# viniciusvidal2/slam-sensor-fusion

Measured on AMD Instinct MI355X. Metric: scans_per_s_200k_scan_vs_10M_map, higher is better.
Workload: dtype f32 points / f64 accumulation

## Files before the change

slam_sensor_fusion_amd/csrc/sf_icp.hip:

```cpp
#include "sf_common.hpp"
#include "sf_nn.hpp"
#include "sf_tile.hpp"
#include "sf_order.hpp"
#include "sf_p2p.hpp"
#include "sf_schedule.hpp"

#include <cfloat>
#include <cstdlib>
#include <cmath>
#include <vector>
#include <mutex>
#include <string>

namespace {

constexpr int BLK = 256;
constexpr int NREC_P2P = 17;
constexpr int NREC_PLANE = 30;
constexpr int REC_STRIDE = 32;

struct IcpState {
    double T[16];
    double rec[REC_STRIDE];
    double fitness, rmse, prev_fitness, prev_rmse;
// ... 454 lines not shown
            }
        }
    }
    return need;
}

struct QueryIn {
    double sx, sy, sz;
    float qx, qy, qz;
    float4 c1, c2;
    float e;
    size_t o;
    bool valid;
};

template <int MODE, bool SHARD>
__device__ __forceinline__ QueryIn query_in(const float *__restrict__ X0x, const float *__restrict__ X0y, const float *__restrict__ X0z, int n, int b, const IcpState *S, float xlo,
                                            float xhi, const uint32_t *__restrict__ own_off, const float4 *__restrict__ qcache, int64_t cache_n, bool cache_live, int slot,
                                            int n_live)
{
    QueryIn q;
    q.sx = q.sy = q.sz = 0.0;
    q.qx = q.qy = q.qz = 0.0f;
    q.c1 = q.c2 = make_float4(0.f, 0.f, 0.f, 0.f);
    q.e = 0.0f;
    q.o = 0;
    q.valid = false;
    if (slot < n_live) {
        const size_t o = SHARD ? (size_t)own_off[b] + (size_t)slot : (size_t)b * n + (size_t)slot;
        q.o = o;
        if (cache_live) {
            q.c1 = qcache[o];
            if (MODE == 2) { q.c2 = qcache[(size_t)cache_n + o]; q.e = q.c2.w; }
            else q.e = reinterpret_cast<const float *>(qcache + (size_t)cache_n)[o];
        }
        const double x0 = X0x[o], y0 = X0y[o], z0 = X0z[o];
        q.sx = S->T[0] * x0 + S->T[1] * y0 + S->T[2] * z0 + S->T[3];
        q.sy = S->T[4] * x0 + S->T[5] * y0 + S->T[6] * z0 + S->T[7];
        q.sz = S->T[8] * x0 + S->T[9] * y0 + S->T[10] * z0 + S->T[11];
        q.qx = (float)q.sx; q.qy = (float)q.sy; q.qz = (float)q.sz;
        q.valid = !SHARD || (q.qx >= xlo && q.qx < xhi);
    }
    return q;
}

__device__ __forceinline__ LanePair make_pair(const QueryIn &q, const sf::NNHit &hit, const float4 &tn)
{
    LanePair P;
    P.sx = q.sx; P.sy = q.sy; P.sz = q.sz;
    P.px = hit.px; P.py = hit.py; P.pz = hit.pz;
    P.tn = tn;
    P.ok = hit.j >= 0;
    return P;
}

template <int MODE>
__device__ __forceinline__ int table_serve(const SfGrid &g, const QueryIn &q, float thr, float m_now, const sf::NNHit &seed, float4 *__restrict__ qcache, int64_t cache_n,
                                            sf::NNHit &hit, float4 &tn)
{
    sf::NNHit th;
    const int stage = sf::nn_research_table(g, q.qx, q.qy, q.qz, thr, seed, th);
    if (stage == 0) return 0;
    const bool same = th.j == seed.j;
    hit = th;
    if (MODE == 2) tn = same ? make_float4(q.c2.x, q.c2.y, q.c2.z, 0.0f) : (th.j >= 0 ? g.nrm[th.j] : make_float4(0.f, 0.f, 0.f, 0.f));
    const float en = fmaxf(sqrtf(th.lb2) * 0.9999f + m_now * 0.999998f - 1.0e-6f, 1.0e-30f);
    if (!same) qcache[q.o] = make_float4(th.px, th.py, th.pz, __int_as_float(th.j));
    if (MODE == 2) qcache[(size_t)cache_n + q.o] = make_float4(tn.x, tn.y, tn.z, en);
    else reinterpret_cast<float *>(qcache + (size_t)cache_n)[q.o] = en;
    return stage;
}

__device__ __forceinline__ void table_count(uint32_t *__restrict__ stats, bool tried, int stage)
{
    const unsigned long long tm = __ballot(tried), sm = __ballot(stage != 0), gm = __ballot(stage == sf::NBR_BY_GAP);
    if ((threadIdx.x & 63) == 0 && tm) {
        uint32_t *sh = stats + NN_STATS_PER * ((blockIdx.x + blockIdx.y * gridDim.x) & (NN_STATS_SHARDS - 1));
        atomicAdd(&sh[2], (uint32_t)__popcll(sm));
        atomicAdd(&sh[3], (uint32_t)__popcll(tm & ~sm));
        atomicAdd(&sh[4], (uint32_t)__popcll(gm));
    }
}

template <int MODE, bool WINDOW, bool SHARD>
__device__ __forceinline__ LanePair nn_pair(const SfGrid &g, const SfWindow &w, const float *__restrict__ X0x, const float *__restrict__ X0y, const float *__restrict__ X0z,
                                            int n, int b, const IcpState *S, float thr, float xlo, float xhi, const uint32_t *__restrict__ own_off,
                                            float4 *__restrict__ qcache, int64_t cache_n, int slot, int n_live, sf::WaveNN *ws, uint32_t *__restrict__ stats,
                                            sf::PhaseClock *pc = nullptr, bool try_table = true)
{
    const bool cache_live = qcache != nullptr && S->cache_live != 0;
    const QueryIn q = query_in<MODE, SHARD>(X0x, X0y, X0z, n, b, S, xlo, xhi, own_off, qcache, cache_n, cache_live, slot, n_live);
    const float qx = q.qx, qy = q.qy, qz = q.qz;
    const size_t o = q.o;
    float *ecache = reinterpret_cast<float *>(qcache + (size_t)cache_n);
    const float m_now = (float)S->motion;
    sf::NNHit hit;
    float4 tn;
    sf::NNHit seed;
    bool need = reuse_certificate(q.valid, qx, qy, qz, thr, m_now, q.e, q.c1, q.c2, hit, tn, seed);
    if constexpr (!WINDOW && !SHARD) {
        if (try_table && g.nbr != nullptr && S->n_research >= g.nbr_from) {
            const bool tried = need && seed.j >= 0;
            int served = 0;
            if (tried) {
                served = table_serve<MODE>(g, q, thr, m_now, seed, qcache, cache_n, hit, tn);
                need = served == 0;
            }
            if (stats) table_count(stats, tried, served);
        }
    }
    const unsigned long long need_mask = __ballot(need);
    if (stats && (threadIdx.x & 63) == 0 && need_mask) {
        uint32_t *sh = stats + NN_STATS_PER * ((blockIdx.x + blockIdx.y * gridDim.x) & (NN_STATS_SHARDS - 1));
        atomicAdd(&sh[0], (uint32_t)__popcll(need_mask));
        atomicAdd(&sh[1], 1u);
    }
    SF_PH(pc, 0);
    if (need_mask != 0ull) {
        const sf::NNHit h = sf::nn_search_wave<WINDOW>(g, w, need, qx, qy, qz, thr, ws, seed, pc);
        if (need) {
            hit = h;
            if (MODE == 2 && h.j >= 0) tn = g.nrm[h.j];
            if (qcache) {
                const float en = fmaxf(sqrtf(h.lb2) * 0.9999f + m_now * 0.999998f - 1.0e-6f, 1.0e-30f);
                qcache[o] = make_float4(h.px, h.py, h.pz, __int_as_float(h.j));
                if (MODE == 2) qcache[(size_t)cache_n + o] = make_float4(tn.x, tn.y, tn.z, en);
                else ecache[o] = en;
            }
        }
    }
    if (qcache && !cache_live && !need && slot < n_live) {
        if (MODE == 2) qcache[(size_t)cache_n + o] = make_float4(0.f, 0.f, 0.f, 0.f);
        else ecache[o] = 0.0f;
    }
    SF_PH(pc, 6);
    return make_pair(q, hit, tn);
}

struct PairTerms { double wgt, ux, uy, uz, tx, ty, tz, ex, ey, ez, d2, r; double J[6]; };
template <int MODE>
__device__ __forceinline__ PairTerms pair_terms(const LanePair &P)
{
    PairTerms t;
    const bool ok = P.ok;
    t.wgt = ok ? 1.0 : 0.0;
    t.ux = ok ? P.sx : 0.0; t.uy = ok ? P.sy : 0.0; t.uz = ok ? P.sz : 0.0;
    t.tx = (double)(ok ? P.px : 0.0f); t.ty = (double)(ok ? P.py : 0.0f); t.tz = (double)(ok ? P.pz : 0.0f);
    t.ex = t.ux - t.tx; t.ey = t.uy - t.ty; t.ez = t.uz - t.tz;
    t.d2 = t.ex * t.ex + t.ey * t.ey + t.ez * t.ez;
    if (MODE == 2) {
        const double nx = (double)(ok ? P.tn.x : 0.0f), ny = (double)(ok ? P.tn.y : 0.0f), nz = (double)(ok ? P.tn.z : 0.0f);
        t.r = t.ex * nx + t.ey * ny + t.ez * nz;
        t.J[0] = t.uy * nz - t.uz * ny; t.J[1] = t.uz * nx - t.ux * nz; t.J[2] = t.ux * ny - t.uy * nx;
        t.J[3] = nx; t.J[4] = ny; t.J[5] = nz;
    } else {
        t.r = 0.0;
#pragma unroll
        for (int a = 0; a < 6; ++a) t.J[a] = 0.0;
    }
    return t;
}

struct RobustArg { int kind; double k; };
__device__ __forceinline__ double robust_weight(const RobustArg &rk, double r)
{
    const double a = fabs(r), k = rk.k;
    switch (rk.kind) {
    case SF_ROBUST_HUBER: return a <= k ? 1.0 : k / a;
    case SF_ROBUST_CAUCHY: { const double q = r / k; return 1.0 / (1.0 + q * q); }
    case SF_ROBUST_TUKEY: { const double q = r / k, s = 1.0 - q * q; return a <= k ? s * s : 0.0; }
    case SF_ROBUST_GM: { const double k2 = k * k, s = k2 / (k2 + r * r); return s * s; }
    default: return 1.0;
    }
}

template <int MODE>
__device__ __forceinline__ void add_half(const PairTerms &t, int h, double (&v)[16])
{
    if (MODE == 1) {
        if (h == 0) {
            v[0] += t.wgt;
            v[1] += t.ux; v[2] += t.uy; v[3] += t.uz;
            v[4] += t.tx; v[5] += t.ty; v[6] += t.tz;
            v[7] = fma(t.ux, t.tx, v[7]); v[8] = fma(t.ux, t.ty, v[8]); v[9] = fma(t.ux, t.tz, v[9]);
            v[10] = fma(t.uy, t.tx, v[10]); v[11] = fma(t.uy, t.ty, v[11]); v[12] = fma(t.uy, t.tz, v[12]);
            v[13] = fma(t.uz, t.tx, v[13]); v[14] = fma(t.uz, t.ty, v[14]); v[15] = fma(t.uz, t.tz, v[15]);
        } else {
            v[0] += t.d2;
        }
    } else {
        if (h == 0) { v[0] += t.wgt; v[1] = fma(t.r, t.r, v[1]); }
        int k = 2;
#pragma unroll
        for (int a = 0; a < 6; ++a) {
#pragma unroll
            for (int c = a; c < 6; ++c) {
                if (h == 0 && k < 16) v[k] = fma(t.J[a], t.J[c], v[k]);
                if (h == 1 && k >= 16) v[k - 16] = fma(t.J[a], t.J[c], v[k - 16]);
                ++k;
            }
        }
        if (h == 1) {
// ... 723 lines not shown
__device__ __forceinline__ constexpr int k6(int a, int b) { return a <= b ? (a == 0 ? b : (a == 1 ? 2 + b : 5)) : (b == 0 ? a : (b == 1 ? 2 + a : 5)); }

struct MomIn { double x[3], n[3], p[3], c, w; };
__device__ __forceinline__ MomIn mom_in(const LanePair &P, bool take)
{
    MomIn t;
    const bool ok = P.ok && take;
    t.w = ok ? 1.0 : 0.0;
    t.x[0] = ok ? P.sx : 0.0; t.x[1] = ok ? P.sy : 0.0; t.x[2] = ok ? P.sz : 0.0;
    t.p[0] = (double)(ok ? P.px : 0.0f); t.p[1] = (double)(ok ? P.py : 0.0f); t.p[2] = (double)(ok ? P.pz : 0.0f);
    t.n[0] = (double)(ok ? P.tn.x : 0.0f); t.n[1] = (double)(ok ? P.tn.y : 0.0f); t.n[2] = (double)(ok ? P.tn.z : 0.0f);
    t.c = t.n[0] * t.p[0] + t.n[1] * t.p[1] + t.n[2] * t.p[2];
    return t;
}
template <int I>
__device__ __forceinline__ double mom_fma(const MomIn &t, double acc)
{
    if constexpr (I < 36) return fma(t.n[k6a(I / 6)] * t.n[k6b(I / 6)], t.x[k6a(I % 6)] * t.x[k6b(I % 6)], acc);
    else if constexpr (I < 54) return fma(t.n[k6a((I - 36) / 3)] * t.n[k6b((I - 36) / 3)], t.x[(I - 36) % 3], acc);
    else if constexpr (I < 60) return fma(t.n[k6a(I - 54)], t.n[k6b(I - 54)], acc);
    else if constexpr (I < 69) return fma(t.c * t.n[(I - 60) / 3], t.x[(I - 60) % 3], acc);
    else if constexpr (I < 72) return fma(t.c, t.n[I - 69], acc);
    else if constexpr (I == 72) return fma(t.c, t.c, acc);
    else if constexpr (I == 73) return acc + t.w;
    else if constexpr (I < 80) return fma(t.x[k6a(I - 74)], t.x[k6b(I - 74)], acc);
    else if constexpr (I < 83) return acc + t.x[I - 80];
    else if constexpr (I < 92) return fma(t.p[(I - 83) / 3], t.x[(I - 83) % 3], acc);
    else if constexpr (I < 95) return acc + t.p[I - 92];
    else return fma(t.p[0], t.p[0], fma(t.p[1], t.p[1], fma(t.p[2], t.p[2], acc)));
}
template <int H, int K = 0>
__device__ __forceinline__ void mom_add16(const MomIn &t, double (&v)[16])
{
    if constexpr (K < 16) {
        v[K] = mom_fma<16 * H + K>(t, v[K]);
        mom_add16<H, K + 1>(t, v);
    }
}

template <bool SHARD>
__device__ __forceinline__ bool stays_frozen(const QueryIn &q, bool in_range, float thr, float m_now, float guard, float xlo, float xhi)
{
    if (!in_range) return true;
    if (!(isfinite(q.qx) && isfinite(q.qy) && isfinite(q.qz))) return true;
    if (SHARD) {
        const float gx = guard * 1.000002f + (fabsf(q.qx) + 1.0f) * 2.6e-7f + 1.0e-6f;
        if (q.valid) {
            if (!(q.qx - gx >= xlo && q.qx + gx < xhi)) return false;
        } else {
            return q.qx + gx < xlo || q.qx - gx >= xhi;
        }
    }
    if (!(q.e > 0.0f)) return false;
    const float m = m_now + guard * 1.000002f;
    const float reach = q.e - m * 1.000002f - (fabsf(q.qx) + fabsf(q.qy) + fabsf(q.qz) + 3.0f * guard + 1.0f) * 2.6e-7f - (q.e + m) * 5.0e-7f - 1.0e-6f;
    const float rt = sqrtf(thr);
    const int32_t jc = __float_as_int(q.c1.w);
    if (jc < 0) return rt * 1.0001f + 1.0e-6f < reach;
    const float d = sqrtf(sf::l2_simple(q.qx, q.qy, q.qz, q.c1.x, q.c1.y, q.c1.z));
    if (!((d + guard) * 1.0001f + 1.0e-6f < reach)) return false;
    const bool stays_in = (d + guard) * 1.0001f + 1.0e-6f < rt * 0.9999f;
    const bool stays_out = (d - guard) * 0.9999f - 1.0e-6f > rt * 1.0001f;
    return stays_in || stays_out;
}

struct FzArgs {
    const float *X0x, *X0y, *X0z;
    int n;
    const IcpState *st;
    float thr, xlo, xhi;
    double *partials;
    int nblocks;
    const uint32_t *own_off;
    float4 *qcache;
    int64_t cache_n;
    uint32_t *stats;
    const FreezeState *fz;
    double *mom_part;
    uint32_t *act_cnt;
    uint16_t *act_ids;
    const uint32_t *act_all;
};

template <int Q, bool SHARD>
__device__ __forceinline__ void nn_red_fz_row(const SfGrid &g, const SfWindow &w, const FzArgs &A, int b, int bx, int fmode)
{
    constexpr int MODE = 2;
    constexpr int NREC = NREC_PLANE;
    static_assert(FZ_CAP == 64 * Q, "wave 0 takes FZ_CAP active queries in Q rounds of 64");
    const float *__restrict__ X0x = A.X0x, *__restrict__ X0y = A.X0y, *__restrict__ X0z = A.X0z;
    const int n = A.n, nblocks = A.nblocks;
    const float thr = A.thr, xlo = A.xlo, xhi = A.xhi;
    double *__restrict__ partials = A.partials, *__restrict__ mom_part = A.mom_part;
    const uint32_t *__restrict__ own_off = A.own_off, *__restrict__ act_all = A.act_all;
    float4 *__restrict__ qcache = A.qcache;
    const int64_t cache_n = A.cache_n;
    uint32_t *__restrict__ stats = A.stats, *__restrict__ act_cnt = A.act_cnt;
    uint16_t *__restrict__ act_ids = A.act_ids;
    const FreezeState *__restrict__ fz = A.fz;
    const IcpState *S = A.st + b;
    const int n_live = SHARD ? (int)(own_off[b + 1] - own_off[b]) : n;
    const int wv = threadIdx.x >> 6, lane = threadIdx.x & 63;
    const size_t row = (size_t)b * nblocks + bx;
    double *dst = partials + row * REC_STRIDE;
    __shared__ sf::WaveNN nn_ws[BLK / 64];
    LanePair P[Q];
    if (fmode == 2) {
        const int64_t total = fz[b].n_active, first = (int64_t)bx * FZ_CAP;
        if (first >= total) return;
        __shared__ double fstage[Q][32];
        if (wv < Q) {
            const uint32_t cnt = (uint32_t)min<int64_t>(total - first, FZ_CAP);
            const uint32_t *list = act_all + (size_t)b * nblocks * FZ_CAP + (size_t)first;
            const uint32_t i = (uint32_t)(wv * 64 + lane);
            const int slot = i < cnt ? (int)list[i] : n_live;
            const LanePair A1 = nn_pair<MODE, false, SHARD>(g, w, X0x, X0y, X0z, n, b, S, thr, xlo, xhi, own_off, qcache, cache_n, slot, n_live, &nn_ws[wv], stats);
#pragma unroll
            for (int h = 0; h < 2; ++h) {
                double v[16];
#pragma unroll
                for (int k = 0; k < 16; ++k) v[k] = 0.0;
                const PairTerms t = pair_terms<MODE>(A1);
                add_half<MODE>(t, h, v);
                const double t0 = wave_reduce_16(v);
                if ((lane & 3) == 0) fstage[wv][16 * h + (lane >> 2)] = t0;
            }
        }
        __syncthreads();
        if (threadIdx.x < NREC) {
            double v = fstage[0][threadIdx.x];
#pragma unroll
            for (int u = 1; u < Q; ++u) v += fstage[u][threadIdx.x];
            dst[threadIdx.x] = v;
        }
        return;
    }
    if (SHARD && bx * (BLK * Q) >= n_live) return;
    __shared__ double stage[BLK / 64][32];
    __shared__ uint32_t act_w[BLK / 64][Q];
    bool active[Q];
#pragma unroll
    for (int u = 0; u < Q; ++u) active[u] = false;
    bool fast = false;
    const float m_now = (float)S->motion;
    const float guard = fz[b].guard;
    const bool attempted = qcache != nullptr && S->cache_live != 0;
    if (attempted) {
        bool any_need = false;
#pragma unroll
        for (int u = 0; u < Q; ++u) {
            const int slot = bx * (BLK * Q) + u * BLK + (int)threadIdx.x;
            const QueryIn q = query_in<MODE, SHARD>(X0x, X0y, X0z, n, b, S, xlo, xhi, own_off, qcache, cache_n, true, slot, n_live);
            sf::NNHit hit, seed;
            float4 tn;
            any_need = reuse_certificate(q.valid, q.qx, q.qy, q.qz, thr, m_now, q.e, q.c1, q.c2, hit, tn, seed) || any_need;
            P[u] = make_pair(q, hit, tn);
            if (fmode == 1) active[u] = !stays_frozen<SHARD>(q, slot < n_live, thr, m_now, guard, xlo, xhi);
        }
        fast = __ballot(any_need) == 0ull;
    }
    if (!fast) {
        asm volatile("" ::: "memory");
#pragma unroll
        for (int u = 0; u < Q; ++u) {
            const int slot = bx * (BLK * Q) + u * BLK + (int)threadIdx.x;
            P[u] = nn_pair<MODE, false, SHARD>(g, w, X0x, X0y, X0z, n, b, S, thr, xlo, xhi, own_off, qcache, cache_n, slot, n_live, &nn_ws[wv], stats);
            if (fmode == 1 && !attempted) active[u] = slot < n_live;
        }
    }
    if (fmode == 1) {
#pragma unroll
        for (int u = 0; u < Q; ++u) {
            const unsigned long long bal = __ballot(active[u]);
            if (lane == 0) act_w[wv][u] = (uint32_t)__popcll(bal);
        }
        __syncthreads();
        uint32_t total = 0;
#pragma unroll
        for (int u = 0; u < Q; ++u) {
            uint32_t base = 0;
#pragma unroll
            for (int ww = 0; ww < BLK / 64; ++ww) {
                if (ww < wv) base += act_w[ww][u];
                total += act_w[ww][u];
            }
            uint32_t before = 0;
#pragma unroll
            for (int uu = 0; uu < Q; ++uu)
                if (uu < u)
#pragma unroll
                    for (int ww = 0; ww < BLK / 64; ++ww) before += act_w[ww][uu];
            const unsigned long long bal = __ballot(active[u]);
            const uint32_t rank = (uint32_t)__builtin_amdgcn_mbcnt_hi((uint32_t)(bal >> 32), __builtin_amdgcn_mbcnt_lo((uint32_t)bal, 0u));
            const uint32_t pos = before + base + rank;
            if (active[u] && pos < (uint32_t)FZ_CAP) act_ids[row * FZ_CAP + pos] = (uint16_t)(u * BLK + (int)threadIdx.x);
        }
        if (threadIdx.x == 0) act_cnt[row] = total;
    }
    bool wave_has_pairs = true;
    if (fmode == 1) {
        bool any = false;
#pragma unroll
        for (int u = 0; u < Q; ++u) any = any || (P[u].ok && active[u]);
        wave_has_pairs = __ballot(any) != 0ull;
        if (!wave_has_pairs && lane < 32) stage[wv][lane] = 0.0;
    }
    if (wave_has_pairs)
#pragma unroll
    for (int h = 0; h < 2; ++h) {
        double v[16];
#pragma unroll
        for (int k = 0; k < 16; ++k) v[k] = 0.0;
#pragma unroll
        for (int u = 0; u < Q; ++u) {
            LanePair A = P[u];
            if (fmode == 1) A.ok = A.ok && active[u];
            const PairTerms t = pair_terms<MODE>(A);
            add_half<MODE>(t, h, v);
        }
        const double t0 = wave_reduce_16(v);
        if ((lane & 3) == 0) stage[wv][16 * h + (lane >> 2)] = t0;
    }
    __syncthreads();
    if (threadIdx.x < NREC) {
        const int c = threadIdx.x;
        dst[c] = ((stage[0][c] + stage[1][c]) + stage[2][c]) + stage[3][c];
    }
    if (fmode != 1) return;
    __shared__ double mstage[BLK / 64][FZ_NMOM];
#define SF_FZ_CHUNK(H)                                                     \
    {                                                                      \
        double v[16];                                                      \
        _Pragma("unroll") for (int k = 0; k < 16; ++k) v[k] = 0.0;         \
        _Pragma("unroll") for (int u = 0; u < Q; ++u)                      \
        {                                                                  \
            const MomIn t = mom_in(P[u], !active[u]);                      \
            mom_add16<H>(t, v);                                            \
        }                                                                  \
        const double t0 = wave_reduce_16(v);                               \
        if ((lane & 3) == 0) mstage[wv][16 * H + (lane >> 2)] = t0;        \
    }
    SF_FZ_CHUNK(0) SF_FZ_CHUNK(1) SF_FZ_CHUNK(2) SF_FZ_CHUNK(3) SF_FZ_CHUNK(4) SF_FZ_CHUNK(5)
#undef SF_FZ_CHUNK
    __syncthreads();
    if (threadIdx.x < FZ_NMOM) {
        const int c = threadIdx.x;
        mom_part[row * FZ_NMOM + c] = ((mstage[0][c] + mstage[1][c]) + mstage[2][c]) + mstage[3][c];
    }
}

template <int Q, bool SHARD>
__global__ __launch_bounds__(BLK, NN_RED_WAVES) void k_nn_red_fz(SfGrid g, SfWindow w, FzArgs A)
{
    const int L = blockIdx.y * gridDim.x + blockIdx.x;
    const int kk = L >> 3;
    const int b = kk % (int)gridDim.y;
    const int bx = (L & 7) * ((int)gridDim.x >> 3) + kk / (int)gridDim.y;
    if (bx >= A.nblocks) return;
    if (A.st[b].done) return;
    nn_red_fz_row<Q, SHARD>(g, w, A, b, bx, A.fz[b].mode);
}

constexpr int FZ_FEW = 16;
template <int Q, bool SHARD>
__global__ __launch_bounds__(BLK, NN_RED_WAVES) void k_nn_red_fz_few(SfGrid g, SfWindow w, FzArgs A)
{
    const int r = (int)blockIdx.x, b = (int)blockIdx.y;
    if (A.st[b].done) return;
    const int fmode = A.fz[b].mode;
    if (fmode == 2) {
        const int64_t total = A.fz[b].n_active;
        for (int bx = r; (int64_t)bx * FZ_CAP < total; bx += FZ_FEW) {
            nn_red_fz_row<Q, SHARD>(g, w, A, b, bx, 2);
            __syncthreads();
        }
        return;
    }
    for (int bx = r; bx < A.nblocks; bx += FZ_FEW) {
        nn_red_fz_row<Q, SHARD>(g, w, A, b, bx, fmode);
        __syncthreads();
    }
}


#ifndef SF_DF_WCAP
#define SF_DF_WCAP 8
#endif
constexpr int DF_WCAP = SF_DF_WCAP;
constexpr int DF_CAPPED = 255;
constexpr int DF_STAT_LAUNCHES = 32;
static_assert((BLK / 64) * DF_WCAP <= FZ_CAP && DF_WCAP < DF_CAPPED, "a row defers fewer queries than it could list as active");
struct DeferBufs {
    uint8_t *cnt;
    uint16_t *ids;
    double *part;
    uint32_t *stat;
};

template <int Q>
__global__ __launch_bounds__(BLK, NN_RED_WAVES) void k_nn_red_df(SfGrid g, SfWindow w, const float *__restrict__ X0x, const float *__restrict__ X0y, const float *__restrict__ X0z,
                                                                 int n, const IcpState *__restrict__ st, float thr, double *__restrict__ partials, int nblocks,
                                                                 float4 *__restrict__ qcache, int64_t cache_n, uint32_t *__restrict__ stats, DeferBufs df, int attempt_from)
{
    constexpr int MODE = 2;
    constexpr int NREC = NREC_PLANE;
    const int L = blockIdx.y * gridDim.x + blockIdx.x;
    const int kk = L >> 3;
    const int b = kk % (int)gridDim.y;
    const int bx = (L & 7) * ((int)gridDim.x >> 3) + kk / (int)gridDim.y;
    if (bx >= nblocks) return;
    const IcpState *S = st + b;
    if (S->done) return;
    __shared__ sf::WaveNN nn_ws[BLK / 64];
    __shared__ double stage[BLK / 64][32];
    const int wv = threadIdx.x >> 6, lane = threadIdx.x & 63;
    const size_t seg = ((size_t)b * nblocks + bx) * (BLK / 64) + wv;
    LanePair P[Q];
    bool need[Q];
#pragma unroll
    for (int u = 0; u < Q; ++u) need[u] = false;
    const bool attempted = qcache != nullptr && S->cache_live != 0 && S->n_research >= attempt_from;
    bool fast = false;
    uint32_t listed = 0;
    if (attempted) {
        const float m_now = (float)S->motion;
#pragma unroll
        for (int u = 0; u < Q; ++u) {
            const int slot = bx * (BLK * Q) + u * BLK + (int)threadIdx.x;
            const QueryIn q = query_in<MODE, false>(X0x, X0y, X0z, n, b, S, 0.0f, 0.0f, nullptr, qcache, cache_n, true, slot, n);
            sf::NNHit hit, seed;
            float4 tn;
            need[u] = reuse_certificate(q.valid, q.qx, q.qy, q.qz, thr, m_now, q.e, q.c1, q.c2, hit, tn, seed);
            if (g.nbr != nullptr && S->n_research >= g.nbr_from) {
                const bool tried = need[u] && seed.j >= 0;
                int served = 0;
                if (tried) {
                    served = table_serve<MODE>(g, q, thr, m_now, seed, qcache, cache_n, hit, tn);
                    need[u] = served == 0;
                }
                if (stats) table_count(stats, tried, served);
            }
            P[u] = make_pair(q, hit, tn);
        }
        uint32_t failing = 0;
#pragma unroll
        for (int u = 0; u < Q; ++u) failing += (uint32_t)__popcll(__ballot(need[u]));
        fast = failing <= (uint32_t)DF_WCAP;
        listed = fast ? failing : (uint32_t)DF_CAPPED;
    }
    if (lane == 0) df.cnt[seg] = (uint8_t)listed;
    if (fast && listed != 0u) {
        uint32_t before = 0;
#pragma unroll
        for (int u = 0; u < Q; ++u) {
            const unsigned long long bal = __ballot(need[u]);
            const uint32_t rank = (uint32_t)__builtin_amdgcn_mbcnt_hi((uint32_t)(bal >> 32), __builtin_amdgcn_mbcnt_lo((uint32_t)bal, 0u));
            if (need[u]) df.ids[seg * DF_WCAP + before + rank] = (uint16_t)(u * BLK + (int)threadIdx.x);
            before += (uint32_t)__popcll(bal);
        }
    }
    if (!fast) {
        asm volatile("" ::: "memory");
// ... 3173 lines not shown
```

slam_sensor_fusion_amd/csrc/sf_nn.hpp:

```cpp
#pragma once
#include "sf_common.hpp"

namespace sf {

#ifdef SF_PHASE_TRACE
constexpr int PH_SLOTS = 16, PH_SHARDS = 64;
struct PhaseClock {
    unsigned long long t;
    unsigned acc[PH_SLOTS];
    __device__ __forceinline__ void start() { for (int i = 0; i < PH_SLOTS; ++i) acc[i] = 0; t = __builtin_amdgcn_s_memtime(); }
    __device__ __forceinline__ void mark(int i) { const unsigned long long n = __builtin_amdgcn_s_memtime(); acc[i] += (unsigned)(n - t); t = n; }
    __device__ __forceinline__ void count(int i, unsigned v) { acc[i] += v; }
};
#define SF_PH(pc, i) do { if (pc) (pc)->mark(i); } while (0)
#define SF_PHC(pc, i, v) do { if (pc) (pc)->count(i, v); } while (0)
#else
struct PhaseClock {};
#define SF_PH(pc, i) do { } while (0)
#define SF_PHC(pc, i, v) do { } while (0)
#endif

struct NNHit {
    float d2;
    int j;
// ... 197 lines not shown
                auto row_cell = [&](int k) -> size_t {
                    const int dy = (int)((OYP >> (2 * k)) & 3u) - 1, dz = (int)((OZP >> (2 * k)) & 3u) - 1;
                    return ((size_t)(cz + dz) * ny + (cy + dy)) * nx + cx;
                };
                {
                    const RowBounds rb = load_row_bounds(g, ((size_t)cz * ny + cy) * nx + cx);
                    scan_row<WINDOW>(g, w, rb, 0.0f, gxm2, gxp2, xm, xp, qx, qy, qz, hit);
                }
                uint32_t mask = 0;
#pragma unroll
                for (int k = 0; k < 8; ++k) {
                    const int dy = (int)((OYP >> (2 * k)) & 3u) - 1, dz = (int)((OZP >> (2 * k)) & 3u) - 1;
                    const bool inside = (unsigned)(cy + dy) < (unsigned)ny && (unsigned)(cz + dz) < (unsigned)nz;
                    if (inside && row_gap2(k) * 0.998f < hit.d2) mask |= 1u << k;
                }
                int k = -1;
                RowBounds cur = {0, 0, 0, 0};
                if (mask) {
                    k = __ffs((int)mask) - 1;
                    mask &= mask - 1;
                    cur = load_row_bounds(g, row_cell(k));
                }
                while (k >= 0) {
                    int k1 = -1;
                    RowBounds nxt = cur;
                    while (mask) {
                        const int kk = __ffs((int)mask) - 1;
                        mask &= mask - 1;
                        if (row_gap2(kk) * 0.998f < hit.d2) {
                            k1 = kk;
                            nxt = load_row_bounds(g, row_cell(kk));
                            break;
                        }
                    }
                    const float g2 = row_gap2(k);
                    if (g2 * 0.998f < hit.d2) scan_row<WINDOW>(g, w, cur, g2, gxm2, gxp2, xm, xp, qx, qy, qz, hit);
                    k = k1;
                    cur = nxt;
                }
            } else {
                for (int z = z0; z <= z1; ++z) {
                    const float rz = safe_gap(cell_gap(gz, z, cz) * h, g.gap_eps);
                    for (int y = y0; y <= y1; ++y) {
                        const float ry = safe_gap(cell_gap(gy, y, cy) * h, g.gap_eps);
                        if ((ry * ry + rz * rz) * 0.998f >= hit.d2) continue;
                        const size_t row = ((size_t)z * ny + y) * nx;
                        scan_range<WINDOW>(g, w, g.cell_start[row + x0], g.cell_start[row + x1 + 1], qx, qy, qz, hit);
                    }
                }
            }
        }
        const float m = block_face_gap(g, gx, gy, gz, cx, cy, cz, R);
        if (m >= 3.0e38f) break;
        const float mm = safe_gap(m, g.gap_eps) * 0.999f;
        if (hit.d2 <= mm * mm) break;
    }
}

template <bool WINDOW>
__device__ __forceinline__ NNHit nn_search(const SfGrid &g, const SfWindow &w, float qx, float qy, float qz, float thr)
{
    NNHit hit;
    hit.d2 = search_start(thr);
    hit.j = -1;
    hit.px = hit.py = hit.pz = 0.0f;
    hit.lb2 = 0.0f;
    if (!(isfinite(qx) && isfinite(qy) && isfinite(qz)) || g.n == 0) return hit;
    if (WINDOW) {
        const float gap = window_gap(w, qx, qy, qz);
        if (gap * gap > thr) return hit;
    }
    nn_rings<WINDOW>(g, w, qx, qy, qz, 1, hit);
    return hit;
}

#ifndef SF_NN_DEAL_K
#define SF_NN_DEAL_K 2
#endif
constexpr int NN_DEAL_K = SF_NN_DEAL_K;
struct WaveNN {
    unsigned long long best[64];
    uint32_t lb2[64];
    float4 q[64];
    RowBounds rb0[64];
    float gap[5][64];
    unsigned long long cell0[64];
    uint16_t task[64 * 11];
    alignas(4) uint8_t mark[64 * NN_DEAL_K];
};

__device__ __forceinline__ unsigned long long pack_hit(float d2, int j) { return ((unsigned long long)__float_as_uint(d2) << 32) | (unsigned long long)(uint32_t)j; }

struct QueryGeo {
    int cx, cy, cz;
    float gxm2, gxp2;
    float gym, gyp, gzm, gzp;
};

__device__ __forceinline__ QueryGeo query_geo(const SfGrid &g, float qx, float qy, float qz)
{
    QueryGeo G;
    const float gx = (qx - g.org[0]) * g.inv_h, gy = (qy - g.org[1]) * g.inv_h, gz = (qz - g.org[2]) * g.inv_h;
    G.cx = grid_cell(gx, g.dim[0]);
    G.cy = grid_cell(gy, g.dim[1]);
    G.cz = grid_cell(gz, g.dim[2]);
    const float h = g.h;
    const float fx = gx - (float)G.cx, fy = gy - (float)G.cy, fz = gz - (float)G.cz;
    const float ge = g.gap_eps;
    const float gxm = safe_gap(fx * h, ge), gxp = safe_gap((1.0f - fx) * h, ge);
    G.gxm2 = G.cx > 0 ? gxm * gxm : 3.0e38f;
    G.gxp2 = G.cx < g.dim[0] - 1 ? gxp * gxp : 3.0e38f;
    G.gym = safe_gap(fy * h, ge);
    G.gyp = safe_gap((1.0f - fy) * h, ge);
    G.gzm = safe_gap(fz * h, ge);
    G.gzp = safe_gap((1.0f - fz) * h, ge);
    return G;
}

__device__ __forceinline__ int row_dy(int k) { return (int)((0x8858u >> (2 * k)) & 3u) - 1; }
__device__ __forceinline__ int row_dz(int k) { return (int)((0xa085u >> (2 * k)) & 3u) - 1; }

__device__ __forceinline__ float row_gap2(const QueryGeo &G, int k)
{
    const int dy = row_dy(k), dz = row_dz(k);
    const float ry = dy < 0 ? G.gym : (dy > 0 ? G.gyp : 0.0f);
    const float rz = dz < 0 ? G.gzm : (dz > 0 ? G.gzp : 0.0f);
    return ry * ry + rz * rz;
}

template <bool MAX>
__device__ __forceinline__ uint32_t wave_incl_scan(uint32_t v)
{
    auto op = [](uint32_t a, uint32_t b) { return MAX ? max(a, b) : a + b; };
    v = op(v, (uint32_t)__builtin_amdgcn_update_dpp(0, (int)v, 0x111, 0xf, 0xf, false));
    v = op(v, (uint32_t)__builtin_amdgcn_update_dpp(0, (int)v, 0x112, 0xf, 0xf, false));
    v = op(v, (uint32_t)__builtin_amdgcn_update_dpp(0, (int)v, 0x114, 0xf, 0xf, false));
    v = op(v, (uint32_t)__builtin_amdgcn_update_dpp(0, (int)v, 0x118, 0xf, 0xf, false));
    v = op(v, (uint32_t)__builtin_amdgcn_update_dpp(0, (int)v, 0x142, 0xa, 0xf, false));
    v = op(v, (uint32_t)__builtin_amdgcn_update_dpp(0, (int)v, 0x143, 0xc, 0xf, false));
    return v;
}

__device__ __forceinline__ void wave_sync()
{
    __builtin_amdgcn_fence(__ATOMIC_ACQ_REL, "wavefront");
    __builtin_amdgcn_wave_barrier();
}

struct RoundTask {
    int owner;
    bool live;
    uint32_t a, b;
    float bound;
    float4 Q;
    unsigned long long start;
};

__device__ __forceinline__ RoundTask round_task(const SfGrid &g, WaveNN *ws, uint32_t e)
{
    const int nx = g.dim[0], ny = g.dim[1];
    RoundTask T;
    T.owner = (int)(e >> 4);
    const int owner = T.owner, t = (int)(e & 15u);
    T.Q = ws->q[owner];
    QueryGeo G;
    G.cx = G.cy = G.cz = 0;
    G.gxm2 = T.Q.w; G.gxp2 = ws->gap[0][owner];
    G.gym = ws->gap[1][owner]; G.gyp = ws->gap[2][owner]; G.gzm = ws->gap[3][owner]; G.gzp = ws->gap[4][owner];
    T.start = __atomic_load_n(&ws->best[owner], __ATOMIC_RELAXED);
    const float cur = __uint_as_float((uint32_t)(T.start >> 32));
    const bool own_row = t < 2 || t == 10;
    const float g2 = own_row ? (t == 0 ? G.gxm2 : (t == 1 ? G.gxp2 : 0.0f)) : row_gap2(G, t - 2);
    T.bound = g2;
    T.a = T.b = 0;
    T.live = g2 * 0.998f < cur;
    if (T.live) {
        T.bound = 3.0e38f;
        if (own_row) {
            const RowBounds rb = ws->rb0[owner];
            T.a = t == 0 ? rb.s0 : (t == 1 ? rb.s2 : rb.s1 + 4);
            T.b = t == 0 ? rb.s1 : (t == 1 ? rb.s3 : rb.s2);
        } else {
            const long long step = ((long long)row_dz(t - 2) * ny + row_dy(t - 2)) * nx;
            const RowBounds rb = load_row_bounds(g, (size_t)((long long)ws->cell0[owner] + step));
            const bool xm = (g2 + G.gxm2) * 0.998f < cur, xp = (g2 + G.gxp2) * 0.998f < cur;
            T.a = xm ? rb.s0 : rb.s1;
            T.b = xp ? rb.s3 : rb.s2;
            if (!xm && rb.s0 < rb.s1) T.bound = g2 + G.gxm2;
            if (!xp && rb.s2 < rb.s3) T.bound = fminf(T.bound, g2 + G.gxp2);
        }
    }
    return T;
}

template <bool WINDOW, bool COOP = false>
__device__ __forceinline__ NNHit nn_search_wave(const SfGrid &g, const SfWindow &w, bool valid, float qx, float qy, float qz, float thr, WaveNN *ws, NNHit seed = NNHit{0.0f, -1, 0.0f, 0.0f, 0.0f, 0.0f},
                                               PhaseClock *pc = nullptr)
{
    const int lane = (int)__lane_id();
    const int nx = g.dim[0], ny = g.dim[1], nz = g.dim[2];
    NNHit hit;
    hit.d2 = search_start(thr);
    hit.j = -1;
    hit.px = hit.py = hit.pz = 0.0f;
    hit.lb2 = 3.0e38f;
    valid = valid && isfinite(qx) && isfinite(qy) && isfinite(qz) && g.n > 0;
    if (WINDOW && valid) {
        const float gap = window_gap(w, qx, qy, qz);
        if (gap * gap > thr) {
            hit.lb2 = gap * gap;
            valid = false;
        }
    }
    if (valid) {
        const float ox = fmaxf(fmaxf(g.org[0] - qx, qx - (g.org[0] + (float)nx * g.h)), 0.0f);
        const float oy = fmaxf(fmaxf(g.org[1] - qy, qy - (g.org[1] + (float)ny * g.h)), 0.0f);
        const float oz = fmaxf(fmaxf(g.org[2] - qz, qz - (g.org[2] + (float)nz * g.h)), 0.0f);
        const float gap = fmaxf(sqrtf(ox * ox + oy * oy + oz * oz) * 0.9995f - 1.0e-3f, 0.0f);
        if (gap * gap > thr) {
            hit.lb2 = gap * gap;
            valid = false;
        }
    }
    if (valid && seed.j >= 0 && seed.d2 < thr) { hit.d2 = seed.d2; hit.j = seed.j; hit.px = seed.px; hit.py = seed.py; hit.pz = seed.pz; }
    uint32_t mask = 0;
    float q_gxm2 = 0.0f;
#ifdef SF_PHASE_TRACE
    QueryGeo G{};
    RowBounds rb0{0, 0, 0, 0};
    if (valid) {
        G = query_geo(g, qx, qy, qz);
        rb0 = load_row_bounds(g, ((size_t)G.cz * ny + G.cy) * nx + G.cx);
        ws->rb0[lane] = rb0;
    }
    SF_PH(pc, 1);
    if (valid && rb0.s1 < rb0.s2) scan4<WINDOW, true>(g, w, rb0.s1, rb0.s2, qx, qy, qz, hit);
    SF_PH(pc, 2);
    if (valid) {
#else
    if (valid) {
        const QueryGeo G = query_geo(g, qx, qy, qz);
        const RowBounds rb0 = load_row_bounds(g, ((size_t)G.cz * ny + G.cy) * nx + G.cx);
        ws->rb0[lane] = rb0;
        if (rb0.s1 < rb0.s2) scan4<WINDOW, true>(g, w, rb0.s1, rb0.s2, qx, qy, qz, hit);
#endif
        if (rb0.s1 + 4 < rb0.s2) {
            if (hit.d2 > 0.0f) mask |= 1u << 10;
            else hit.lb2 = 0.0f;
        }
        if (rb0.s0 < rb0.s1) {
            if (G.gxm2 * 0.998f < hit.d2) mask |= 1u;
            else hit.lb2 = fminf(hit.lb2, G.gxm2);
        }
        if (rb0.s2 < rb0.s3) {
            if (G.gxp2 * 0.998f < hit.d2) mask |= 2u;
            else hit.lb2 = fminf(hit.lb2, G.gxp2);
        }
#pragma unroll
        for (int k = 0; k < 8; ++k) {
            const bool inside = (unsigned)(G.cy + row_dy(k)) < (unsigned)ny && (unsigned)(G.cz + row_dz(k)) < (unsigned)nz;
            const float gap2 = row_gap2(G, k);
            if (inside) {
                if (gap2 * 0.998f < hit.d2) mask |= 4u << k;
                else hit.lb2 = fminf(hit.lb2, gap2);
            }
        }
        if (mask) {
            q_gxm2 = G.gxm2;
            ws->gap[0][lane] = G.gxp2;
            ws->gap[1][lane] = G.gym; ws->gap[2][lane] = G.gyp; ws->gap[3][lane] = G.gzm; ws->gap[4][lane] = G.gzp;
            ws->cell0[lane] = ((unsigned long long)G.cz * (unsigned long long)ny + (unsigned long long)G.cy) * (unsigned long long)nx + (unsigned long long)G.cx;
        }
    }
    ws->best[lane] = pack_hit(hit.d2, hit.j);
    ws->lb2[lane] = __float_as_uint(hit.lb2);
    ws->q[lane] = make_float4(qx, qy, qz, q_gxm2);
    int total = 0;
#pragma unroll
    for (int t = 0; t < 11; ++t) {
        const bool has = (mask >> t) & 1u;
        const unsigned long long bal = __ballot(has);
        const int rank = (int)__builtin_amdgcn_mbcnt_hi((uint32_t)(bal >> 32), __builtin_amdgcn_mbcnt_lo((uint32_t)bal, 0u));
        if (has) ws->task[total + rank] = (uint16_t)((lane << 4) | t);
        total += __popcll(bal);
    }
    __builtin_amdgcn_fence(__ATOMIC_ACQ_REL, "wavefront");
    __builtin_amdgcn_wave_barrier();
    SF_PH(pc, 3);
    SF_PHC(pc, 11, (unsigned)total);
#ifdef SF_PHASE_TRACE
    unsigned lane_trips = 0, lane_cands = 0;
#endif
    for (int i0 = 0; i0 < total; i0 += 64) {
        SF_PHC(pc, 9, 1u);
        const int idx = i0 + lane;
        if constexpr (WINDOW) {
#ifdef SF_PHASE_TRACE
            unsigned my_trips = 0;
#endif
            if (idx < total) {
                const RoundTask T = round_task(g, ws, ws->task[idx]);
                float bound = T.bound;
                if (T.live) {
                    NNHit h;
                    h.d2 = __uint_as_float((uint32_t)(T.start >> 32));
                    h.j = (int)(uint32_t)T.start;
                    h.px = h.py = h.pz = 0.0f;
                    h.lb2 = 3.0e38f;
                    scan_range<WINDOW, true>(g, w, T.a, T.b, T.Q.x, T.Q.y, T.Q.z, h);
#ifdef SF_PHASE_TRACE
                    my_trips = (T.b - T.a + 3u) / 4u; lane_cands += T.b - T.a; lane_trips += my_trips;
#endif
                    bound = fminf(bound, h.lb2);
                    const unsigned long long mine = pack_hit(h.d2, h.j);
                    if (mine != T.start) {
                        const unsigned long long old = atomicMin(&ws->best[T.owner], mine);
                        bound = fminf(bound, __uint_as_float((uint32_t)((old > mine ? old : mine) >> 32)));
                    }
                }
                atomicMin(&ws->lb2[T.owner], __float_as_uint(bound));
            }
#ifdef SF_PHASE_TRACE
            { unsigned m = my_trips; for (int o = 32; o > 0; o >>= 1) m = max(m, (unsigned)__shfl_xor((int)m, o)); SF_PHC(pc, 10, m); }
#endif
        } else {
            uint32_t a = 0, len = 0;
            int owner = 0;
            if (idx < total) {
                const RoundTask T = round_task(g, ws, ws->task[idx]);
                owner = T.owner;
                if (T.live) { a = T.a; len = T.b - T.a; }
                atomicMin(&ws->lb2[owner], __float_as_uint(T.bound));
            }
            const uint32_t incl = wave_incl_scan<false>(len);
            const uint32_t off = incl - len;
            const uint32_t tot = (uint32_t)__builtin_amdgcn_readlane((int)incl, 63);
            const uint32_t base = a - off;
            SF_PHC(pc, 13, tot);
            uint32_t carry = 0;
            for (uint32_t c0 = 0; c0 < tot; c0 += 64u * NN_DEAL_K) {
                SF_PHC(pc, 10, 1u);
                for (int i = lane; i < 16 * NN_DEAL_K; i += 64) reinterpret_cast<uint32_t *>(ws->mark)[i] = 0u;
                __builtin_amdgcn_wave_barrier();
                if (len != 0u && off - c0 < 64u * NN_DEAL_K && off >= c0) ws->mark[off - c0] = (uint8_t)(lane + 1);
                wave_sync();
                uint32_t src[NN_DEAL_K];
#pragma unroll
                for (int k = 0; k < NN_DEAL_K; ++k) src[k] = wave_incl_scan<true>((uint32_t)ws->mark[64 * k + lane]);
#pragma unroll
                for (int k = 0; k < NN_DEAL_K; ++k) {
                    src[k] = max(src[k], carry);
                    carry = (uint32_t)__builtin_amdgcn_readlane((int)src[k], 63);
                }
                wave_sync();
                SF_PHC(pc, 12, (unsigned)__popcll(__ballot(c0 + (uint32_t)lane < tot)));
                uint32_t j[NN_DEAL_K];
                int ow[NN_DEAL_K];
                float4 p[NN_DEAL_K], Q[NN_DEAL_K];
                unsigned long long cur[NN_DEAL_K];
#pragma unroll
                for (int k = 0; k < NN_DEAL_K; ++k) {
                    const uint32_t s = c0 + 64u * (uint32_t)k + (uint32_t)lane;
                    const int from = (int)((src[k] - 1u) & 63u) << 2;
                    j[k] = (uint32_t)__builtin_amdgcn_ds_bpermute(from, (int)base) + s;
                    ow[k] = __builtin_amdgcn_ds_bpermute(from, owner);
                    p[k] = load_point(g, j[k], s < tot);
                }
#pragma unroll
                for (int k = 0; k < NN_DEAL_K; ++k) {
                    Q[k] = ws->q[ow[k]];
                    cur[k] = __atomic_load_n(&ws->best[ow[k]], __ATOMIC_RELAXED);
                }
#pragma unroll
                for (int k = 0; k < NN_DEAL_K; ++k) {
                    const bool live = c0 + 64u * (uint32_t)k + (uint32_t)lane < tot;
// ... 193 lines not shown
```

Baseline: 22110.

## Add wide-round wave NN search that processes own-row tasks first, then batched neighbor rows

```diff
diff --git a/slam_sensor_fusion_amd/csrc/sf_icp.hip b/slam_sensor_fusion_amd/csrc/sf_icp.hip
--- a/slam_sensor_fusion_amd/csrc/sf_icp.hip
+++ b/slam_sensor_fusion_amd/csrc/sf_icp.hip
@@ -560,7 +560,7 @@
     }
 }
 
-template <int MODE, bool WINDOW, bool SHARD>
+template <int MODE, bool WINDOW, bool SHARD, int FORM = sf::NN_ROUNDS_WIDE>
 __device__ __forceinline__ LanePair nn_pair(const SfGrid &g, const SfWindow &w, const float *__restrict__ X0x, const float *__restrict__ X0y, const float *__restrict__ X0z,
                                             int n, int b, const IcpState *S, float thr, float xlo, float xhi, const uint32_t *__restrict__ own_off,
                                             float4 *__restrict__ qcache, int64_t cache_n, int slot, int n_live, sf::WaveNN *ws, uint32_t *__restrict__ stats,
@@ -595,7 +595,7 @@
     }
     SF_PH(pc, 0);
     if (need_mask != 0ull) {
-        const sf::NNHit h = sf::nn_search_wave<WINDOW>(g, w, need, qx, qy, qz, thr, ws, seed, pc);
+        const sf::NNHit h = sf::nn_search_wave<WINDOW, false, FORM>(g, w, need, qx, qy, qz, thr, ws, seed, pc);
         if (need) {
             hit = h;
             if (MODE == 2 && h.j >= 0) tn = g.nrm[h.j];
@@ -1485,7 +1485,7 @@
     const uint32_t *act_all;
 };
 
-template <int Q, bool SHARD>
+template <int Q, bool SHARD, int FORM = sf::NN_ROUNDS_WIDE>
 __device__ __forceinline__ void nn_red_fz_row(const SfGrid &g, const SfWindow &w, const FzArgs &A, int b, int bx, int fmode)
 {
     constexpr int MODE = 2;
@@ -1517,7 +1517,7 @@
             const uint32_t *list = act_all + (size_t)b * nblocks * FZ_CAP + (size_t)first;
             const uint32_t i = (uint32_t)(wv * 64 + lane);
             const int slot = i < cnt ? (int)list[i] : n_live;
-            const LanePair A1 = nn_pair<MODE, false, SHARD>(g, w, X0x, X0y, X0z, n, b, S, thr, xlo, xhi, own_off, qcache, cache_n, slot, n_live, &nn_ws[wv], stats);
+            const LanePair A1 = nn_pair<MODE, false, SHARD, FORM>(g, w, X0x, X0y, X0z, n, b, S, thr, xlo, xhi, own_off, qcache, cache_n, slot, n_live, &nn_ws[wv], stats);
 #pragma unroll
             for (int h = 0; h < 2; ++h) {
                 double v[16];
@@ -1567,7 +1567,7 @@
 #pragma unroll
         for (int u = 0; u < Q; ++u) {
             const int slot = bx * (BLK * Q) + u * BLK + (int)threadIdx.x;
-            P[u] = nn_pair<MODE, false, SHARD>(g, w, X0x, X0y, X0z, n, b, S, thr, xlo, xhi, own_off, qcache, cache_n, slot, n_live, &nn_ws[wv], stats);
+            P[u] = nn_pair<MODE, false, SHARD, FORM>(g, w, X0x, X0y, X0z, n, b, S, thr, xlo, xhi, own_off, qcache, cache_n, slot, n_live, &nn_ws[wv], stats);
             if (fmode == 1 && !attempted) active[u] = slot < n_live;
         }
     }
@@ -1674,13 +1674,13 @@
     if (fmode == 2) {
         const int64_t total = A.fz[b].n_active;
         for (int bx = r; (int64_t)bx * FZ_CAP < total; bx += FZ_FEW) {
-            nn_red_fz_row<Q, SHARD>(g, w, A, b, bx, 2);
+            nn_red_fz_row<Q, SHARD, sf::NN_ROUNDS_FIXED>(g, w, A, b, bx, 2);
             __syncthreads();
         }
         return;
     }
     for (int bx = r; bx < A.nblocks; bx += FZ_FEW) {
-        nn_red_fz_row<Q, SHARD>(g, w, A, b, bx, fmode);
+        nn_red_fz_row<Q, SHARD, sf::NN_ROUNDS_FIXED>(g, w, A, b, bx, fmode);
         __syncthreads();
     }
 }
diff --git a/slam_sensor_fusion_amd/csrc/sf_nn.hpp b/slam_sensor_fusion_amd/csrc/sf_nn.hpp
--- a/slam_sensor_fusion_amd/csrc/sf_nn.hpp
+++ b/slam_sensor_fusion_amd/csrc/sf_nn.hpp
@@ -303,7 +303,10 @@
     unsigned long long best[64];
     uint32_t lb2[64];
     float4 q[64];
-    RowBounds rb0[64];
+    union {
+        RowBounds rb0[64];
+        uint32_t base[128];
+    };
     float gap[5][64];
     unsigned long long cell0[64];
     uint16_t task[64 * 11];
@@ -414,7 +417,154 @@
     return T;
 }
 
-template <bool WINDOW, bool COOP = false>
+constexpr int NN_ROUNDS_FIXED = 0, NN_ROUNDS_WIDE = 1;
+constexpr int NN_TASKS_OWN = 0, NN_TASKS_ROWS = 1;
+#ifndef SF_NN_ROW_K
+#define SF_NN_ROW_K 2
+#endif
+constexpr int NN_ROW_K = SF_NN_ROW_K;
+static_assert(NN_ROW_K == 1 || NN_ROW_K == 2, "mark[] holds the task slot + 1 in a byte");
+
+template <int KIND>
+__device__ __forceinline__ constexpr bool task_own_row() { return KIND == NN_TASKS_OWN; }
+
+template <int KIND>
+__device__ __forceinline__ float task_gap2(const WaveNN *ws, int owner, int t)
+{
+    if (task_own_row<KIND>()) {
+        const float v = t == 0 ? ws->q[owner].w : ws->gap[0][owner];
+        return t == 10 ? 0.0f : v;
+    }
+    const int dy = row_dy(t - 2), dz = row_dz(t - 2);
+    const float ry = dy != 0 ? ws->gap[dy < 0 ? 1 : 2][owner] : 0.0f;
+    const float rz = dz != 0 ? ws->gap[dz < 0 ? 3 : 4][owner] : 0.0f;
+    return ry * ry + rz * rz;
+}
+
+template <int K, int KIND>
+__device__ __forceinline__ void wide_rounds(const SfGrid &g, WaveNN *ws, const int lane, int head, const int end, PhaseClock *pc)
+{
+    constexpr uint32_t NONE = 0xffffffffu, XM = 1u << 16, XP = 1u << 17;
+    const int nx = g.dim[0], ny = g.dim[1];
+    for (; head < end; head += 64 * K) {
+        const int head0 = head;
+        SF_PHC(pc, KIND == NN_TASKS_OWN ? 9 : 12, 1u);
+        uint32_t e[K];
+        float bm[K], bp[K];
+        RowBounds rb[K];
+#pragma unroll
+        for (int u = 0; u < K; ++u) {
+            e[u] = NONE;
+            bm[u] = bp[u] = 3.0e38f;
+            rb[u] = RowBounds{0u, 0u, 0u, 0u};
+            const int idx = head0 + 64 * u + lane;
+            if (idx < end) {
+                const uint32_t x = ws->task[idx];
+                const int owner = (int)(x >> 4), t = (int)(x & 15u);
+                const float cur = __uint_as_float((uint32_t)(__atomic_load_n(&ws->best[owner], __ATOMIC_RELAXED) >> 32));
+                const float g2 = task_gap2<KIND>(ws, owner, t);
+                if (task_own_row<KIND>()) {
+                    const RowBounds r0 = ws->rb0[owner];
+                    if (g2 * 0.998f < cur) { e[u] = x; rb[u] = r0; }
+                } else {
+                    const float gxm2 = ws->q[owner].w, gxp2 = ws->gap[0][owner];
+                    const long long step = ((long long)row_dz(t - 2) * ny + row_dy(t - 2)) * nx;
+                    const size_t cell = (size_t)((long long)ws->cell0[owner] + step);
+                    if (g2 * 0.998f < cur) {
+                        e[u] = x;
+                        if ((g2 + gxm2) * 0.998f < cur) e[u] |= XM; else bm[u] = g2 + gxm2;
+                        if ((g2 + gxp2) * 0.998f < cur) e[u] |= XP; else bp[u] = g2 + gxp2;
+                        rb[u] = load_row_bounds(g, cell);
+                    }
+                }
+                if (e[u] == NONE) atomicMin(&ws->lb2[owner], __float_as_uint(g2));
+            }
+#ifdef SF_PHASE_TRACE
+            SF_PHC(pc, 15, (unsigned)__popcll(__ballot(idx < end && e[u] == NONE)));
+#endif
+        }
+        static_assert(K == 1 || KIND == NN_TASKS_ROWS, "rb0 is free only once the own-row tasks are done");
+        uint32_t base = 0u, off[K], tot = 0u;
+#pragma unroll
+        for (int u = 0; u < K; ++u) {
+            uint32_t a = 0u, len = 0u;
+            if (e[u] != NONE) {
+                const int owner = (int)((e[u] >> 4) & 63u), t = (int)(e[u] & 15u);
+                if (task_own_row<KIND>()) {
+                    a = t == 0 ? rb[u].s0 : (t == 1 ? rb[u].s2 : rb[u].s1 + 4u);
+                    len = (t == 0 ? rb[u].s1 : (t == 1 ? rb[u].s3 : rb[u].s2)) - a;
+                } else {
+                    const bool xm = (e[u] & XM) != 0u, xp = (e[u] & XP) != 0u;
+                    a = xm ? rb[u].s0 : rb[u].s1;
+                    len = (xp ? rb[u].s3 : rb[u].s2) - a;
+                    const float bound = fminf(rb[u].s0 < rb[u].s1 ? bm[u] : 3.0e38f, rb[u].s2 < rb[u].s3 ? bp[u] : 3.0e38f);
+                    if (bound < 3.0e38f) atomicMin(&ws->lb2[owner], __float_as_uint(bound));
+                }
+            }
+            const uint32_t incl = wave_incl_scan<false>(len);
+            off[u] = tot + incl - len;
+            base = a - off[u];
+            if (K > 1) ws->base[64 * u + lane] = base;
+            if (len == 0u) off[u] = NONE;
+            tot += (uint32_t)__builtin_amdgcn_readlane((int)incl, 63);
+        }
+        SF_PHC(pc, 13, tot);
+        uint32_t carry = 0;
+        for (uint32_t c0 = 0; c0 < tot; c0 += 64u * NN_DEAL_K) {
+            SF_PHC(pc, 10, 1u);
+            for (int i = lane; i < 16 * NN_DEAL_K; i += 64) reinterpret_cast<uint32_t *>(ws->mark)[i] = 0u;
+            __builtin_amdgcn_wave_barrier();
+#pragma unroll
+            for (int u = 0; u < K; ++u)
+                if (off[u] != NONE && off[u] >= c0 && off[u] - c0 < 64u * NN_DEAL_K) ws->mark[off[u] - c0] = (uint8_t)(64 * u + lane + 1);
+            wave_sync();
+            uint32_t src[NN_DEAL_K];
+#pragma unroll
+            for (int k = 0; k < NN_DEAL_K; ++k) src[k] = wave_incl_scan<true>((uint32_t)ws->mark[64 * k + lane]);
+#pragma unroll
+            for (int k = 0; k < NN_DEAL_K; ++k) {
+                src[k] = max(src[k], carry);
+                carry = (uint32_t)__builtin_amdgcn_readlane((int)src[k], 63);
+            }
+            wave_sync();
+            uint32_t j[NN_DEAL_K];
+            int ow[NN_DEAL_K];
+            float4 p[NN_DEAL_K], Q[NN_DEAL_K];
+            unsigned long long cur[NN_DEAL_K];
+#pragma unroll
+            for (int k = 0; k < NN_DEAL_K; ++k) {
+                const uint32_t s = c0 + 64u * (uint32_t)k + (uint32_t)lane;
+                const uint32_t slot = (src[k] - 1u) & (64u * K - 1u);
+                const int from = (int)(slot & 63u) << 2;
+                j[k] = (K > 1 ? ws->base[slot] : (uint32_t)__builtin_amdgcn_ds_bpermute(from, (int)base)) + s;
+                ow[k] = src[k] != 0u ? (int)((ws->task[head0 + (int)slot] >> 4) & 63u) : 0;
+                p[k] = load_point(g, j[k], s < tot);
+            }
+#pragma unroll
+            for (int k = 0; k < NN_DEAL_K; ++k) {
+                Q[k] = ws->q[ow[k]];
+                cur[k] = __atomic_load_n(&ws->best[ow[k]], __ATOMIC_RELAXED);
+            }
+#pragma unroll
+            for (int k = 0; k < NN_DEAL_K; ++k) {
+                const bool live = c0 + 64u * (uint32_t)k + (uint32_t)lane < tot;
+                const float d2 = l2_simple(Q[k].x, Q[k].y, Q[k].z, p[k].x, p[k].y, p[k].z);
+                const unsigned long long mine = pack_hit(d2, (int)j[k]);
+                if (live && mine != cur[k]) {
+                    uint32_t lose = __float_as_uint(d2);
+                    if (mine < cur[k]) {
+                        const unsigned long long old = atomicMin(&ws->best[ow[k]], mine);
+                        lose = (uint32_t)((old > mine ? old : mine) >> 32);
+                    }
+                    atomicMin(&ws->lb2[ow[k]], lose);
+                }
+            }
+        }
+        wave_sync();
+    }
+}
+
+template <bool WINDOW, bool COOP = false, int FORM = NN_ROUNDS_WIDE>
 __device__ __forceinline__ NNHit nn_search_wave(const SfGrid &g, const SfWindow &w, bool valid, float qx, float qy, float qz, float thr, WaveNN *ws, NNHit seed = NNHit{0.0f, -1, 0.0f, 0.0f, 0.0f, 0.0f},
                                                PhaseClock *pc = nullptr)
 {
@@ -496,14 +646,17 @@
     ws->best[lane] = pack_hit(hit.d2, hit.j);
     ws->lb2[lane] = __float_as_uint(hit.lb2);
     ws->q[lane] = make_float4(qx, qy, qz, q_gxm2);
-    int total = 0;
-#pragma unroll
-    for (int t = 0; t < 11; ++t) {
+    constexpr bool OWN_FIRST = !WINDOW && FORM == NN_ROUNDS_WIDE;
+    int total = 0, n_own = 0;
+#pragma unroll
+    for (int i = 0; i < 11; ++i) {
+        const int t = OWN_FIRST ? (i < 2 ? i : (i == 2 ? 10 : i - 1)) : i;
         const bool has = (mask >> t) & 1u;
         const unsigned long long bal = __ballot(has);
         const int rank = (int)__builtin_amdgcn_mbcnt_hi((uint32_t)(bal >> 32), __builtin_amdgcn_mbcnt_lo((uint32_t)bal, 0u));
         if (has) ws->task[total + rank] = (uint16_t)((lane << 4) | t);
         total += __popcll(bal);
+        if (i == 2) n_own = total;
     }
     __builtin_amdgcn_fence(__ATOMIC_ACQ_REL, "wavefront");
     __builtin_amdgcn_wave_barrier();
@@ -512,6 +665,10 @@
 #ifdef SF_PHASE_TRACE
     unsigned lane_trips = 0, lane_cands = 0;
 #endif
+    if constexpr (OWN_FIRST) {
+        wide_rounds<1, NN_TASKS_OWN>(g, ws, lane, 0, n_own, pc);
+        wide_rounds<NN_ROW_K, NN_TASKS_ROWS>(g, ws, lane, n_own, total, pc);
+    } else
     for (int i0 = 0; i0 < total; i0 += 64) {
         SF_PHC(pc, 9, 1u);
         const int idx = i0 + lane;
```

Result: no change. 22060 (median of 2 runs) (-0.2%).
